# TheClimateCorporation/photon-ml

Measured on AMD Instinct MI355X. Metric: examples/sec/node, logistic L-BFGS 1B×1M-sparse, higher is better.
Workload: dtype bf16; 1 GPU; model=logistic_regression_l2_lbfgs, global_batch=125000000, rows_per_gpu=125000000, features=1000000, nnz_per_row=100, parallelism=dp1, optimizer_state=replicated, layout=tiled

## Files before the change

### photon_ml_amd/ops/csrc/game_kernels.hip

```cpp

#include <hip/hip_runtime.h>
#include <stdint.h>

#include <algorithm>

#ifndef PML_BUILD_ID
#define PML_BUILD_ID "unstamped-build!"
#endif
__attribute__((used)) static const char pml_build_stamp[] = "PML_BUILD_ID=" PML_BUILD_ID;

#define LAUNCH_CHECK()                                         \
  do {                                                         \
    hipError_t e_ = hipGetLastError();                         \
    if (e_ != hipSuccess) return (int)e_;                      \
  } while (0)

#define SCORE_GROUP 16
#define SCORE_THREADS 256
#define SCORE_ROWS_PER_BLOCK (SCORE_THREADS / SCORE_GROUP)

template <bool RE>
__global__ __launch_bounds__(SCORE_THREADS) void score_rows_kernel(
    const long long* __restrict__ indptr, const int* __restrict__ col, const double* __restrict__ val,
    long long n_rows, const double* __restrict__ w, const int* __restrict__ ent,
// ... 90 lines not shown
    for (long long p = lo; p < hi; ++p) {
      const double v = val[p];
      const long long c = col[p];
      if (j < k) acc += v * PT[c * k + j];
    }
    if (j < k) Y[row * k + j] = acc;
  }
}

__device__ __forceinline__ unsigned long long splitmix64(unsigned long long x) {
  x += 0x9E3779B97F4A7C15ull;
  x = (x ^ (x >> 30)) * 0xBF58476D1CE4E5B9ull;
  x = (x ^ (x >> 27)) * 0x94D049BB133111EBull;
  return x ^ (x >> 31);
}

template <typename T>
__global__ __launch_bounds__(256) void downsample_kernel(const T* __restrict__ y, const T* __restrict__ w0,
                                                          const long long* __restrict__ rowid, long long n,
                                                          unsigned long long seed, double rate, int binary,
                                                          T* __restrict__ w) {
  const long long i = (long long)blockIdx.x * 256 + threadIdx.x;
  if (i >= n) return;
  const unsigned long long id = rowid ? (unsigned long long)rowid[i] : (unsigned long long)i;
  const double u = (double)(splitmix64(seed ^ splitmix64(id)) >> 11) * 0x1.0p-53;
  const double wi = (double)w0[i];
  double out;
  if (binary) {
    const bool pos = (double)y[i] >= 0.5;
    out = pos ? wi : (u < rate ? wi / rate : 0.0);
  } else {
    out = u < rate ? wi : 0.0;
  }
  w[i] = (T)out;
}

#define CMP_SEG 8
struct CmpArgs {
  const int* units;
  int col_e, row_col;
  const int* seg;
  int nseg, sbits, key_is_row;
  const uint32_t* pack;
  const void* val;
  const uint16_t* npack;
  const void* nval;
  const int* nbase;
  const unsigned char* keep;
  int* seg_cnt;
  const long long* seg_first;
  const long long* unit_lo;
  uint32_t* opack;
  void* oval;
};

template <typename VT, int PASS>
__global__ __launch_bounds__(256) void tl_compact_kernel(CmpArgs a) {
  const int lane = threadIdx.x & 63;
  const int s = __builtin_amdgcn_readfirstlane(blockIdx.x * 4 + (threadIdx.x >> 6));
  if (s >= a.nseg) return;
  const int* sg = a.seg + 3 * (long long)s;
  const int u = sg[0], r_lo = sg[1], r_hi = sg[2];
  const int* ut = a.units + 6 * (long long)u;
  const long long e_lo = ut[a.col_e];
  const int nw = ut[a.col_e + 1] - ut[a.col_e];
  const int n_lo = ut[4], nn = ut[5] - ut[4];
  const uint32_t row0 = a.row_col >= 0 ? (uint32_t)ut[a.row_col] : 0u;
  const uint32_t smask = (1u << a.sbits) - 1u;
  const VT* val = (const VT*)a.val;
  const VT* nval = (const VT*)a.nval;
  long long ob = PASS ? a.seg_first[s] : 0;
  const long long olo = PASS ? a.unit_lo[u] : 0;
  const unsigned long long below = (1ull << lane) - 1ull;
  int cnt = 0;
  for (int r = r_lo; r < r_hi; ++r) {
    uint32_t p[4];
    VT v[4];
    bool ok[4];
    if (r < nn) {
      const long long q = (long long)n_lo + r;
      const int base = a.nbase[q];
#pragma unroll
      for (int k = 0; k < 4; ++k) {
        const uint32_t p16 = a.npack[q * 256 + 4 * lane + k];
        p[k] = ((uint32_t)(base + (int)(p16 >> a.sbits)) << a.sbits) | (p16 & smask);
        v[k] = nval[q * 256 + 4 * lane + k];
        ok[k] = true;
      }
    } else {
      const int w = r - nn;
#pragma unroll
      for (int k = 0; k < 4; ++k) {
        ok[k] = 256 * w + 64 * k + lane < nw;
        const long long e = e_lo + 256LL * w + 4 * lane + k;
        p[k] = ok[k] ? a.pack[e] : 0u;
        v[k] = ok[k] ? val[e] : (VT)0;
      }
    }
#pragma unroll
    for (int k = 0; k < 4; ++k) {
      const uint32_t row = a.key_is_row ? (p[k] >> a.sbits) : row0 + (p[k] & smask);
      const bool kp = ok[k] && a.keep[row];
      const unsigned long long m = __ballot(kp);
      if (PASS) {
        if (kp) {
          const long long o = ob + __popcll(m & below);
          const long long ph = olo + (o & ~255LL) + ((o & 63) << 2) + ((o & 255) >> 6);
          a.opack[ph] = p[k];
          ((VT*)a.oval)[ph] = v[k];
        }
        ob += __popcll(m);
      } else {
        cnt += __popcll(m);
      }
    }
  }
  if (!PASS && lane == 0) a.seg_cnt[s] = cnt;
}


template <int S, bool STAGE>
__global__ __launch_bounds__(64) void seg_gram_kernel(int B, int n, int dmax, const long long* __restrict__ ents,
                                                      const long long* __restrict__ row_ptr,
                                                      const long long* __restrict__ col_ptr,
                                                      const long long* __restrict__ nip,
                                                      const long long* __restrict__ pos,
                                                      const double* __restrict__ val, double* __restrict__ K) {
  extern __shared__ double img[];
  const int lane = threadIdx.x;
  const long long b = blockIdx.x;
  if (b >= B) return;
  const long long e = ents[b];
  const long long r0 = row_ptr[e];
  const int ne = (int)(row_ptr[e + 1] - r0);
  const long long cb = col_ptr[e];
  const int de = (int)(col_ptr[e + 1] - cb);
  const long long e0 = nip[r0];
  const int enz = (int)(nip[r0 + ne] - e0);
  double* sval = img + (size_t)dmax * S;
  unsigned short* scol = (unsigned short*)(sval + enz);
  int* sptr = (int*)(scol + ((enz + 3) & ~3));
  for (int c = lane; c < de * S; c += 64) img[c] = 0.0;
  if (STAGE) {
    for (int t = lane; t < enz; t += 64) {
      sval[t] = val[e0 + t];
      scol[t] = (unsigned short)(pos[e0 + t] - cb);
    }
    for (int i = lane; i <= ne; i += 64) sptr[i] = (int)(nip[r0 + i] - e0);
  }
  __syncthreads();
  double* Kb = K + b * (long long)n * n;
  for (int i0 = 0; i0 < ne; i0 += S) {
    const int ns = ne - i0 < S ? ne - i0 : S;
    for (int s = 0; s < ns; ++s) {
      if (STAGE) {
        const int ib = sptr[i0 + s], ie = sptr[i0 + s + 1];
        for (int t = ib + lane; t < ie; t += 64) img[(int)scol[t] * S + s] = sval[t];
      } else {
        const long long ib = nip[r0 + i0 + s], ie = nip[r0 + i0 + s + 1];
        for (long long t = ib + lane; t < ie; t += 64) img[(pos[t] - cb) * S + s] = val[t];
      }
    }
    __syncthreads();
    for (int j = lane; j < n; j += 64) {
      double acc[S];
#pragma unroll
      for (int s = 0; s < S; ++s) acc[s] = 0.0;
      if (j < ne) {
        if (STAGE) {
// ... 330 lines not shown
```

### photon_ml_amd/ops/csrc/glm_kernels.hip

```cpp

#include <hip/hip_runtime.h>
#include <stdint.h>
#include <math.h>
#include <algorithm>

#define NB 4096
#define NTHREADS 256
#define VEC 8
#define MAXSEG 1024

#define LAUNCH_CHECK()                                         \
  do {                                                         \
    hipError_t e_ = hipGetLastError();                         \
    if (e_ != hipSuccess) return (int)e_;                      \
  } while (0)

enum LossId { LOSS_LOGISTIC = 0, LOSS_POISSON = 1, LOSS_SQUARED = 2, LOSS_HINGE = 3 };
enum FwdMode { FWD_MARGIN = 0, FWD_VALUE_GRAD = 1, FWD_HV = 2, FWD_DZZ = 3, FWD_LS = 4 };

struct bf16x8 { uint4 u; };

template <typename VT, typename AT> struct Loader;
template <> struct Loader<uint16_t, float> {
  static __device__ __forceinline__ void load8(const uint16_t* __restrict__ p, float* v) {
// ... 746 lines not shown
typedef const __attribute__((address_space(4))) int* const_int_p;

template <typename VT, typename XT, typename AT, bool SQ, int NW, int S, int D>
__device__ __forceinline__ void tl_stream_ring(const uint32_t* __restrict__ pack, const VT* __restrict__ val,
                                               const XT* __restrict__ x, int e_lo, int e_hi, int sbits, AT* acc,
                                               const int* wbase) {
  constexpr int R = S + 1;
  static_assert(D < S && R % (D + 1) == 0, "gathers run ahead of loaded slots; the gather ring divides the slots");
  typedef typename TLValT<VT>::T LT;
  typedef typename TLVals<VT>::Raw Raw;
  const int lane = threadIdx.x & 63;
  const int w = __builtin_amdgcn_readfirstlane(threadIdx.x >> 6);
  const uint32_t smask = (1u << sbits) - 1u;
  const int nr = (e_hi - e_lo + TL_ROUND - 1) / TL_ROUND;
  const int r0 = (nr * w) / NW, r1 = (nr * (w + 1)) / NW;
  if (r0 >= r1) return;
  v4u pk[R];
  Raw vr[R];
  uint32_t bs[R];
  XT xg[D + 1][TL_VEC];
  const int ws = wbase ? 1 : 0;
  const const_int_p wb = (const_int_p)(wbase ? wbase : g_zero_base);
  const int rb0 = e_lo / TL_ROUND;
  auto load_round = [&](int r, v4u& p, Raw& v, uint32_t& b) {
    const int e = e_lo + min(r, r1 - 1) * TL_ROUND + lane * TL_VEC;
    p = ldg_nt((const v4u*)(pack + e));
    v = TLVals<VT>::load(val + e);
    b = (uint32_t)wb[ws * (rb0 + min(r, r1 - 1))];
  };
  const int abl = TL_ABL;
  AT regsum = AT(0);
  auto gather = [&](int r, const v4u& p, uint32_t b, XT* xv) {
    const int e = e_lo + r * TL_ROUND + lane;
#pragma unroll
    for (int k = 0; k < TL_VEC; ++k) {
      const uint32_t key = (e + 64 * k < e_hi) ? b + (p[k] >> sbits) : 0u;
      const bool hot = key < ((uint32_t)abl >> 8) << 10;
      if (abl & 10) xv[k] = XT(1);
      else if ((abl & 32) && hot) xv[k] = XT(1);
      else if ((abl & 64) && __ballot(!hot) == 0ull) xv[k] = XT(1);
      else xv[k] = ldg(x + key);
    }
  };
#pragma unroll
  for (int i = 0; i < S; ++i) {
    load_round(r0 + i, pk[i], vr[i], bs[i]);
    __builtin_amdgcn_sched_barrier(0);
  }
#pragma unroll
  for (int i = 0; i < D; ++i) {
    gather(r0 + i, pk[i], bs[i], xg[i]);
    __builtin_amdgcn_sched_barrier(0);
  }
  for (int r = r0; r < r1; r += R) {
#pragma unroll
    for (int i = 0; i < R; ++i) {
      const int rc = r + i;
      load_round(rc + S, pk[(i + S) % R], vr[(i + S) % R], bs[(i + S) % R]);
      __builtin_amdgcn_sched_barrier(0);
      gather(rc + D, pk[(i + D) % R], bs[(i + D) % R], xg[(i + D) % (D + 1)]);
      __builtin_amdgcn_sched_barrier(0);
      LT v[TL_VEC];
      TLVals<VT>::get(vr[i], v);
      const int e = e_lo + rc * TL_ROUND + lane;
#pragma unroll
      for (int k = 0; k < TL_VEC; ++k) {
        const bool in = (e + 64 * k < e_hi) && (rc < r1);
        const AT vv = SQ ? static_cast<AT>(v[k]) * static_cast<AT>(v[k]) : static_cast<AT>(v[k]);
        AT add;
        if (abl & 4) add = in ? static_cast<AT>(static_cast<float>(v[k]) * static_cast<float>(xg[i % (D + 1)][k]))
                              : AT(0);
        else add = in ? vv * static_cast<AT>(xg[i % (D + 1)][k]) : AT(0);
        if (abl & 1) regsum += add;
        else atomicAdd(&acc[in ? (pk[i][k] & smask) : 0u], add);
      }
      __builtin_amdgcn_sched_barrier(0);
    }
  }
  if (abl & 1) atomicAdd(&acc[lane], regsum);
}

template <typename T> __device__ __forceinline__ T lane_bcast(T v, int src) { return __shfl(v, src, 64); }

template <typename VT, typename XT, typename AT, bool SQ, int NW, int S = 2>
__device__ __forceinline__ void tl_stream_narrow(const uint16_t* __restrict__ npk, const VT* __restrict__ nvl,
                                                 const int* __restrict__ nbs, int n_lo, int n_hi, int sbits,
                                                 const XT* __restrict__ x, AT* acc) {
  constexpr int R = S + 1;
  typedef typename TLValT<VT>::T LT;
  typedef typename TLVals<VT>::Raw Raw;
  const int lane = threadIdx.x & 63;
  const int w = __builtin_amdgcn_readfirstlane(threadIdx.x >> 6);
  const int nr = n_hi - n_lo;
  const int r0 = n_lo + (nr * w) / NW, r1 = n_lo + (nr * (w + 1)) / NW;
  if (r0 >= r1) return;
  const uint32_t smask = (1u << sbits) - 1u;
  const const_int_p bp = (const_int_p)nbs;
  v2u pks[R];
  Raw vs[R];
  XT xs[R];
  const int abl = TL_ABL;
  AT regsum = AT(0);
  auto issue = [&](int r, int base, v2u& pk, Raw& v, XT& xw) {
    const size_t e = (size_t)min(r, r1 - 1) * TL_ROUND + lane * TL_VEC;
    pk = ldg_nt((const v2u*)(npk + e));
    v = TLVals<VT>::load(nvl + e);
    xw = (abl & 18) ? XT(1) : ldg(x + base + lane);
  };
#pragma unroll
  for (int i = 0; i < S; ++i) {
    issue(r0 + i, bp[min(r0 + i, r1 - 1)], pks[i], vs[i], xs[i]);
    __builtin_amdgcn_sched_barrier(0);
  }
  int nb = bp[min(r0 + S, r1 - 1)];
  for (int r = r0; r < r1; r += R) {
#pragma unroll
    for (int i = 0; i < R; ++i) {
      const int rc = r + i;
      issue(rc + S, nb, pks[(i + S) % R], vs[(i + S) % R], xs[(i + S) % R]);
      nb = bp[min(rc + S + 1, r1 - 1)];
      __builtin_amdgcn_sched_barrier(0);
      const bool live = rc < r1;
      LT v[TL_VEC];
      TLVals<VT>::get(vs[i], v);
      const v2u pk = pks[i];
      const uint32_t p[TL_VEC] = {pk.x & 0xffffu, pk.x >> 16, pk.y & 0xffffu, pk.y >> 16};
#pragma unroll
      for (int k = 0; k < TL_VEC; ++k) {
        const XT xv = (abl & 16) ? xs[i] : lane_bcast(xs[i], (int)(p[k] >> sbits));
        const AT vv = SQ ? static_cast<AT>(v[k]) * static_cast<AT>(v[k]) : static_cast<AT>(v[k]);
        AT add;
        if (abl & 4) add = live ? static_cast<AT>(static_cast<float>(v[k]) * static_cast<float>(xv)) : AT(0);
        else add = live ? vv * static_cast<AT>(xv) : AT(0);
        if (abl & 1) regsum += add + AT(p[k] & smask);
        else atomicAdd(&acc[live ? (p[k] & smask) : 0u], add);
      }
      __builtin_amdgcn_sched_barrier(0);
    }
  }
  if (abl & 1) atomicAdd(&acc[lane], regsum);
}

template <typename VT, typename XT, typename AT, bool SQ, int U, int NW, int P>
__device__ __forceinline__ void tl_stream(const uint32_t* __restrict__ pack, const VT* __restrict__ val,
                                          const XT* __restrict__ x, int e_lo, int e_hi, int sbits, AT* acc,
                                          const int* wbase = nullptr) {
  if (P == 1) tl_stream_p1<VT, XT, AT, SQ, U, NW>(pack, val, x, e_lo, e_hi, sbits, acc);
  else if (P == 2) tl_stream_wide<VT, XT, AT, SQ, NW, 2>(pack, val, x, e_lo, e_hi, sbits, acc);
  else if (P == 3) tl_stream_ring<VT, XT, AT, SQ, NW, 2, 0>(pack, val, x, e_lo, e_hi, sbits, acc, wbase);
  else if (P == 5) tl_stream_ring<VT, XT, AT, SQ, NW, 3, 1>(pack, val, x, e_lo, e_hi, sbits, acc, wbase);
  else if (P == 6) tl_stream_ring<VT, XT, AT, SQ, NW, 5, 2>(pack, val, x, e_lo, e_hi, sbits, acc, wbase);
  else tl_stream_p0<VT, XT, AT, SQ, U, NW>(pack, val, x, e_lo, e_hi, sbits, acc);
}

struct TLNarrow { const uint16_t* pack; const void* val; const int* base; const int* wbase; };

template <typename VT, typename XT, typename RT, typename AT, int MAXR, int U, int NW, int P>
__device__ __forceinline__ void tl_fwd_block(int b, int row_lo, int nrows, int e_lo, int e_hi, int n_lo, int n_hi,
                                             int rbits, const uint32_t* __restrict__ pack,
                                             const VT* __restrict__ val, const TLNarrow& nar,
                                             const XT* __restrict__ x, const FwdArgs<XT, RT>& a,
                                             double* __restrict__ stats, AT (*acc)[MAXR], double* red) {
  const int R = 1 << rbits;
  for (int i = threadIdx.x; i < R; i += NW * 64)
#pragma unroll
    for (int w = 0; w < NW; ++w) acc[w][i] = AT(0);
  __syncthreads();
  if (n_hi > n_lo)
    tl_stream_narrow<VT, XT, AT, false, NW, (P >= 5 ? 4 : 2)>(nar.pack, (const VT*)nar.val, nar.base, n_lo, n_hi,
                                                              rbits, x,
                                            acc[threadIdx.x >> 6]);
  tl_stream<VT, XT, AT, false, U, NW, P>(pack, val, x, e_lo, e_hi, rbits, acc[threadIdx.x >> 6], nar.wbase);
  __syncthreads();
  double F = 0.0, S = 0.0;
  for (int r = threadIdx.x; r < nrows; r += NW * 64) {
    double z = static_cast<double>(acc[0][r]);
#pragma unroll
    for (int w = 1; w < NW; ++w) z += static_cast<double>(acc[w][r]);
    const int s = row_lo + r;
    fwd_finish(a, s, z, fwd_prefetch(a, s), F, S);
  }
  if (stats) {
    block_sum2_nw<NW>(F, S, red);
    if (threadIdx.x == 0) { stats[2 * b] = F; stats[2 * b + 1] = S; }
  }
}

template <typename VT, typename XT, typename RT, typename AT, int MAXR, int U, int NW, int P>
__global__ __launch_bounds__(NW * 64) void tl_fwd_kernel(const int* __restrict__ blk, int rbits,
                                                          const uint32_t* __restrict__ pack,
                                                          const VT* __restrict__ val, TLNarrow nar,
                                                          const XT* __restrict__ x, FwdArgs<XT, RT> a,
                                                          double* __restrict__ stats,
                                                          const unsigned char* __restrict__ live) {
  __shared__ AT acc[NW][MAXR];
  __shared__ double red[2 * NW];
  const int b = blockIdx.x;
  if (live && !live[b]) return;
  const int* q = blk + 6 * b;
  tl_fwd_block<VT, XT, RT, AT, MAXR, U, NW, P>(b, q[0], q[1], q[2], q[3], q[4], q[5], rbits, pack, val, nar, x, a,
                                              stats, acc, red);
}

template <typename VT, typename XT, typename RT, typename AT, int MAXR, int U, int NW, int P>
__global__ __launch_bounds__(NW * 64) void tl_fwd_multi_kernel(const int* __restrict__ blk, int rbits,
                                                                const unsigned long long* __restrict__ ptrs,
                                                                const XT* __restrict__ x, FwdArgs<XT, RT> a,
                                                                double* __restrict__ stats,
                                                                const unsigned char* __restrict__ live) {
  __shared__ AT acc[NW][MAXR];
  __shared__ double red[2 * NW];
  const int b = blockIdx.x;
  if (live && !live[b]) return;
  const int* q = blk + 8 * b;
  const unsigned long long* pc = ptrs + 6 * q[0];
  const TLNarrow nar = {(const uint16_t*)pc[2], (const void*)pc[3], (const int*)pc[4], (const int*)pc[5]};
  tl_fwd_block<VT, XT, RT, AT, MAXR, U, NW, P>(b, q[1], q[2], q[3], q[4], q[6], q[7], rbits, (const uint32_t*)pc[0],
                                              (const VT*)pc[1], nar, x + q[5], a, stats, acc, red);
}

template <typename VT, typename XT, typename AT, bool SQ, int MAXR, int U, int NW, int P>
__device__ __forceinline__ void tl_t_item(int tile, int e_lo, int e_hi, int part, int n_lo, int n_hi, int cbits,
                                          const uint32_t* __restrict__ pack, const VT* __restrict__ val,
                                          const TLNarrow& nar, const XT* __restrict__ x, double* __restrict__ G,
                                          int dim, double* __restrict__ parts, AT (*acc)[MAXR]) {
  const int C = 1 << cbits;
  for (int i = threadIdx.x; i < C; i += NW * 64)
#pragma unroll
    for (int w = 0; w < NW; ++w) acc[w][i] = AT(0);
  __syncthreads();
  if (n_hi > n_lo)
    tl_stream_narrow<VT, XT, AT, SQ, NW, (P >= 5 ? 4 : 2)>(nar.pack, (const VT*)nar.val, nar.base, n_lo, n_hi,
                                                           cbits, x,
                                         acc[threadIdx.x >> 6]);
  tl_stream<VT, XT, AT, SQ, U, NW, P>(pack, val, x, e_lo, e_hi, cbits, acc[threadIdx.x >> 6], nar.wbase);
  __syncthreads();
  const int c0 = tile << cbits;
  for (int c = threadIdx.x; c < C; c += NW * 64) {
    double s = static_cast<double>(acc[0][c]);
#pragma unroll
    for (int w = 1; w < NW; ++w) s += static_cast<double>(acc[w][c]);
    if (part < 0) {
      if (c0 + c < dim) G[c0 + c] += s;
    } else {
      parts[(size_t)part * C + c] = s;
    }
  }
}

template <typename VT, typename XT, typename AT, bool SQ, int MAXR, int U, int NW, int P>
__global__ __launch_bounds__(NW * 64) void tl_t_kernel(const int* __restrict__ items, int cbits,
                                                        const uint32_t* __restrict__ pack,
                                                        const VT* __restrict__ val, TLNarrow nar,
                                                        const XT* __restrict__ x, double* __restrict__ G, int dim,
                                                        double* __restrict__ parts,
                                                        const unsigned char* __restrict__ live) {
  __shared__ AT acc[NW][MAXR];
  if (live && !live[blockIdx.x]) return;
  const int* q = items + 6 * blockIdx.x;
  tl_t_item<VT, XT, AT, SQ, MAXR, U, NW, P>(q[0], q[1], q[2], q[3], q[4], q[5], cbits, pack, val, nar, x, G, dim,
                                            parts, acc);
}

template <typename VT, typename XT, typename AT, bool SQ, int MAXR, int U, int NW, int P>
__global__ __launch_bounds__(NW * 64) void tl_t_multi_kernel(const int* __restrict__ items, int cbits,
                                                              const unsigned long long* __restrict__ ptrs,
                                                              const XT* __restrict__ x, double* __restrict__ G,
                                                              int dim, double* __restrict__ parts,
                                                              const unsigned char* __restrict__ live,
                                                              const int* __restrict__ gate) {
  __shared__ AT acc[NW][MAXR];
  if (gate && *gate == 0) return;
  if (live && !live[blockIdx.x]) return;
  const int* q = items + 8 * blockIdx.x;
  const unsigned long long* pc = ptrs + 6 * q[0];
  const TLNarrow nar = {(const uint16_t*)pc[2], (const void*)pc[3], (const int*)pc[4], (const int*)pc[5]};
  tl_t_item<VT, XT, AT, SQ, MAXR, U, NW, P>(q[1], q[2], q[3], q[4], q[6], q[7], cbits, (const uint32_t*)pc[0],
                                            (const VT*)pc[1], nar, x + q[5], G, dim, parts, acc);
}

__device__ __forceinline__ double rows_sum64(const double* __restrict__ src, int C, int r0, int r1, int c,
                                             double* sh) {
  const int w = threadIdx.x >> 6, lane = threadIdx.x & 63;
  const int n = r1 - r0;
  const int q0 = r0 + (n * w) / 4, q1 = r0 + (n * (w + 1)) / 4;
  double s0 = 0.0, s1 = 0.0, s2 = 0.0, s3 = 0.0;
  if (c < C) {
    int r = q0;
    for (; r + 3 < q1; r += 4) {
      s0 += src[(size_t)r * C + c];
      s1 += src[(size_t)(r + 1) * C + c];
      s2 += src[(size_t)(r + 2) * C + c];
      s3 += src[(size_t)(r + 3) * C + c];
    }
    for (; r < q1; ++r) s0 += src[(size_t)r * C + c];
  }
  sh[w * 64 + lane] = (s0 + s1) + (s2 + s3);
  __syncthreads();
  return (sh[lane] + sh[64 + lane]) + (sh[128 + lane] + sh[192 + lane]);
}

__global__ __launch_bounds__(NTHREADS) void tl_t_combine1_kernel(const int* __restrict__ cu, int cbits,
                                                                 const double* __restrict__ parts,
                                                                 double* __restrict__ l1,
                                                                 const unsigned char* __restrict__ live_mt) {
  __shared__ double sh[NTHREADS];
  const int u = blockIdx.x;
  if (live_mt && !live_mt[cu[3 * u]]) return;
  const int C = 1 << cbits;
  const int c = blockIdx.y * 64 + (threadIdx.x & 63);
  const double s = rows_sum64(parts, C, cu[3 * u + 1], cu[3 * u + 2], c, sh);
  if (threadIdx.x < 64 && c < C) l1[(size_t)u * C + c] = s;
}

__global__ __launch_bounds__(NTHREADS) void tl_t_combine2_kernel(const int* __restrict__ mt_tiles,
                                                                 const int* __restrict__ mt_ptr, int cbits,
                                                                 const double* __restrict__ l1,
// ... 2454 lines not shown
```

### photon_ml_amd/ops/device.py

```python
from __future__ import annotations

import ctypes
import os
import threading
from dataclasses import dataclass
from typing import List, Optional, Sequence

import numpy as np
import scipy.sparse as sp
import torch

from ..data.matrix import LabeledData
from .native import SegChunkDesc, check, require_glm_lib, stream_handle
from .reference import GLMComputable
from .tiled import DEFAULT_ITEM_ENTRIES, TLFwdChunk, TLTChunk, tl_supported
from ..utils.timing import phase, trace_range

H2D_GATE = threading.Event()

LAYOUTS = ("auto", "tiled", "segmented")


def resolve_layout(layout: str, dim: int, chunk_rows: int) -> str:
    import os
# ... 150 lines not shown
        if os.environ.get("PML_CHECK_KERNEL_INPUTS", "0") == "1":
            self.validate()

    def validate(self):
        from .tiled import il_phys
        for c, (f, t) in enumerate(zip(self.csr, self.csc)):
            if f.kind != "tl":
                continue
            m = self.row_starts[c + 1] - self.row_starts[c]
            b = f.blk.cpu().to(torch.int64)
            if f.nblk and (int(b[:, 0].min()) < 0 or int((b[:, 0] + b[:, 1]).max()) > m
                           or int(b[:, 1].max()) > (1 << f.rbits)):
                raise ValueError(f"chunk {c}: forward block rows out of range")
            q = 256 if f.il else 4
            end = b[:, 2] + (b[:, 3] - b[:, 2] + q - 1) // q * q if f.il else (b[:, 3] + 3) // 4 * 4
            if f.nblk and (int(b[:, 2].min()) < 0 or int(end.max()) > f.pack.numel()):
                raise ValueError(f"chunk {c}: forward block window outside the stream")
            if f.il and f.nblk and bool((b[:, 2] % 256 != 0).any()):
                raise ValueError(f"chunk {c}: interleaved forward windows not round-aligned")
            ncols = int(self.dim) - self.col_lo[c]
            self._validate_narrow(c, f, b, ncols, "forward")
            pk, _ = f.logical()
            p = pk.cpu().to(torch.int64)
            wb = getattr(f, "wbase", None)
            if wb is not None and wb.numel() and int(wb.min()) < 0:
                raise ValueError(f"chunk {c}: negative wide-round base")
            if p.numel() and int((p >> f.rbits).max()) >= ncols:
                raise ValueError(f"chunk {c}: forward gather index >= column window")
            counts = f.unit_counts().cpu()
            blk_rows = torch.repeat_interleave(b[:, 1], counts)
            if p.numel() and bool(((p & ((1 << f.rbits) - 1)) >= blk_rows).any()):
                raise ValueError(f"chunk {c}: forward LDS slot >= block rows")
            it = t.items.cpu().to(torch.int64)
            if t.nitems:
                if int(it[:, 1].min()) < 0 or int(it[:, 2].max()) > t.pack.numel():
                    raise ValueError(f"chunk {c}: transpose item window outside the stream")
                if int(it[:, 3].max()) >= max(t.nparts, 1) and t.nparts:
                    raise ValueError(f"chunk {c}: transpose partial-row slot out of range")
                self._validate_narrow(c, t, it, m, "transpose")
                tp, _ = t.logical()
                q = tp.cpu().to(torch.int64) & 0xFFFFFFFF
                if q.numel() and int((q >> t.cbits).max()) >= m:
                    raise ValueError(f"chunk {c}: transpose gather row >= chunk rows")
                cols = (torch.repeat_interleave(it[:, 0], t.unit_counts().cpu()) << t.cbits) + (q & ((1 << t.cbits) - 1))
                if q.numel() and int(cols.max()) >= t.dim:
                    raise ValueError(f"chunk {c}: transpose column >= dim")
        if self.parts.numel() < max([c.parts_needed for c in self.csr + self.csc] + [1]):
            raise ValueError("partial-row scratch too small")
        self._validate_multi()
        return True

    def _validate_multi(self):
        mb = getattr(self, "_multi", None)
        if mb is not None and not isinstance(mb, str):
            t = self._multi_blk.cpu().to(torch.int64)
            for c, ch in enumerate(self.csr):
                r = t[t[:, 0] == c]
                if ch.il and r.shape[0] and (int(r[:, 3].min()) < 0 or int((r[:, 3] + (r[:, 4] - r[:, 3] + 255) // 256 * 256).max())
                                   > ch.pack.numel() or int(r[:, 7].max()) > ch.nbase.numel() * (ch.n_narrow_rounds > 0)):
                    raise ValueError(f"chunk {c}: shard-wide forward table outside the chunk's streams")
        mt = getattr(self, "_multi_t", None)
        if mt is not None and not isinstance(mt, str):
            if self.parts.numel() < mt.parts_needed:
                raise ValueError("partial-row scratch too small for the shard-wide transpose")
            t = mt.items.cpu().to(torch.int64)
            for c, ch in enumerate(self.csc):
                r = t[t[:, 0] == c]
                if ch.il and r.shape[0] and (int(r[:, 2].min()) < 0 or int((r[:, 2] + (r[:, 3] - r[:, 2] + 255) // 256 * 256).max())
                                   > ch.pack.numel() or int(r[:, 7].max()) > ch.nbase.numel() * (ch.n_narrow_rounds > 0)):
                    raise ValueError(f"chunk {c}: shard-wide transpose table outside the chunk's streams")

    @staticmethod
    def _validate_narrow(c: int, ch, table: torch.Tensor, xlen: int, what: str):
        if table.shape[0] == 0:
            return
        n_lo, n_hi = table[:, 4], table[:, 5]
        nrounds = ch.nbase.numel() if ch.n_narrow_rounds else 0
        if bool((n_hi < n_lo).any()) or int(n_hi.max()) > nrounds or bool((n_lo[1:] != n_hi[:-1]).any()):
            raise ValueError(f"chunk {c}: {what} narrow round ranges inconsistent")
        if nrounds:
            base = ch.nbase.cpu().to(torch.int64)
            if ch.npack.numel() < 256 * nrounds or ch.nval.numel() < 256 * nrounds:
                raise ValueError(f"chunk {c}: {what} narrow stream shorter than its rounds")
            if int(base.min()) < 0 or int(base.max()) + 64 > xlen:
                raise ValueError(f"chunk {c}: {what} narrow key window outside the gathered vector")

    @staticmethod
    def from_labeled(data: LabeledData, device="cuda", precision: str = "f64", chunk_rows: int = 1 << 20,
                     relabel: bool = True, layout: str = "auto", item_entries: Optional[int] = None,
                     col_windows: bool = False):
        if col_windows:
            relabel = False
        prec = PRECISIONS[precision]
        vdt = VAL_DTYPE[prec]
        dev = torch.device(device)
        x = data.x.tocsr()
        n, d = x.shape
        if dev.type == "cuda" and n and resolve_layout(layout, d, chunk_rows) == "tiled":
            return DeviceGLMData._from_labeled_device(x, data, dev, precision, chunk_rows, relabel, item_entries,
                                                      col_windows)
        if hasattr(x, "to_scipy"):
            x = x.to_scipy()
        old_of_new = None
        from ..parallel.dist import is_dist
        shared = relabel and is_dist() and not col_windows
        if shared or (relabel and x.nnz > 0):
            counts = np.bincount(x.indices, minlength=d).astype(np.int64)
            if shared:
                import torch.distributed as tdist
                from ..parallel.sharding import comm_device
                ct = torch.from_numpy(counts).to(comm_device())
                tdist.all_reduce(ct)
                counts = ct.cpu().numpy()
            old_of_new_np = np.argsort(-counts, kind="stable")
            new_of_old_np = np.empty(d, dtype=np.int64)
            new_of_old_np[old_of_new_np] = np.arange(d)
            x = sp.csr_matrix((x.data, new_of_old_np[x.indices], x.indptr), shape=x.shape)
            old_of_new = torch.from_numpy(old_of_new_np)
        starts = list(range(0, n, chunk_rows)) + [n]
        if n == 0:
            starts = [0, 0]
        csr, csc = [], []
        col_lo = []
        wins = []
        align = _window_align(chunk_rows, precision)
        for a, b in zip(starts[:-1], starts[1:]):
            xc = x[a:b]
            if col_windows and xc.nnz:
                lo, hi = int(xc.indices.min()), int(xc.indices.max()) + 1
                lo -= lo % align
            else:
                lo, hi = 0, d
            wins.append((lo, hi))
        dmax = max([hi - lo for lo, hi in wins] + [1])
        layout = resolve_layout(layout, dmax, chunk_rows)
        cbits = None
        if layout == "tiled" and not col_windows and item_entries is None:
            from .tiled import shard_t_config
            cbits, item_entries = shard_t_config(int(x.nnz), n, d, chunk_rows)
        for (a, b), (lo, hi) in zip(zip(starts[:-1], starts[1:]), wins):
            xc = x[a:b]
            col_lo.append(lo)
            if lo != 0 or hi != d:
                xc = sp.csr_matrix((xc.data, xc.indices - lo, xc.indptr), shape=(b - a, hi - lo))
            dc = hi - lo
            if layout == "tiled":
                rp = torch.from_numpy((xc.indptr - xc.indptr[0]).astype(np.int64)).to(dev)
                col = torch.from_numpy(xc.indices.astype(np.int64)).to(dev)
                val = torch.from_numpy(xc.data.astype(np.float64)).to(dev).to(vdt)
                csr.append(TLFwdChunk(rp, col, val, dc))
                csc.append(TLTChunk(rp, col, val, dc, chunk_rows, cbits=cbits, item_entries=item_entries))
                continue
            sp_ = (xc.indptr - xc.indptr[0]).astype(np.int32)
            csr.append(SegChunk(sp_, torch.from_numpy(xc.indices.astype(np.int32)),
                                torch.from_numpy(xc.data.astype(np.float64)).to(vdt), dev, forward=True))
            xt = xc.tocsc()
            xt.sort_indices()
            xc = xc.copy()
            csc.append(SegChunk(xt.indptr.astype(np.int32), torch.from_numpy(xt.indices.astype(np.int32)),
                                torch.from_numpy(xt.data.astype(np.float64)).to(vdt), dev))
        out = DeviceGLMData(csr, csc, starts, torch.from_numpy(data.y), torch.from_numpy(data.offsets),
                            torch.from_numpy(data.weights), d, precision, dev, old_of_new)
        out.col_lo = col_lo
        return out

    @staticmethod
# ... 886 lines not shown
```

### photon_ml_amd/ops/tiled.py

```python
from __future__ import annotations

import ctypes
import math
import os
from typing import Optional, Sequence, Tuple

import numpy as np
import torch

from .native import TLFwdDesc, TLTDesc

TL_MAXBITS = 12
TL_MAXBITS_F64 = 11
TL_MINBITS = 5
DEFAULT_RBITS = int(os.environ.get("PML_TL_RBITS", 10))
DEFAULT_CBITS = int(os.environ.get("PML_TL_CBITS", 10))
DEFAULT_ITEM_ENTRIES = 1 << 18
_PAD = 8
COMBINE_SEG = 16


XCD_GROUPS = int(os.environ.get("PML_TL_XCD", "0"))


def xcd_order(chunk_of_item: np.ndarray, groups: int) -> np.ndarray:
    stream = np.asarray(chunk_of_item) % groups
    lists = [np.flatnonzero(stream == k) for k in range(groups)]
    longest = max(len(l) for l in lists)
    grid = np.full((longest, groups), -1, dtype=np.int64)
    for k, l in enumerate(lists):
        grid[: len(l), k] = l
    order = grid.reshape(-1)
    return order[order >= 0]


def combine_seg(k: int) -> int:
    return max(COMBINE_SEG, int(math.ceil(math.sqrt(k))))
IL_ROUND = 256
TL_VEC = 4
INTERLEAVE = int(os.environ.get("PML_TL_IL", "1"))
NARROW = int(os.environ.get("PML_TL_NARROW", "1"))
NARROW_W = 64
WIDE_BASE = int(os.environ.get("PML_TL_WIDE_BASE", "1"))


def narrow_width(sbits: int) -> int:
    return min(NARROW_W, 1 << max(16 - sbits, 0))


def _bits(n: int) -> int:
    return max(1, int(n - 1).bit_length())


def _cap(want: int, f64: bool) -> int:
    return min(want, TL_MAXBITS_F64 if f64 else TL_MAXBITS)


F64_WIDE_RBITS = 11


def default_rbits(dim: int, f64: bool) -> int:
    if f64 and dim >= (1 << 16) and "PML_TL_RBITS" not in os.environ:
        return F64_WIDE_RBITS
    return DEFAULT_RBITS


def fwd_bits(dim: int, f64: bool = False, want: Optional[int] = None) -> Optional[int]:
    r = min(_cap(default_rbits(dim, f64) if want is None else want, f64), 32 - _bits(dim))
    return r if r >= TL_MINBITS else None


def t_bits(chunk_rows: int, f64: bool = False, want: Optional[int] = None) -> Optional[int]:
    c = min(_cap(DEFAULT_CBITS if want is None else want, f64), 32 - _bits(chunk_rows))
    return c if c >= TL_MINBITS else None


SPARSE_TILE_ENTRIES = 1 << 16


def shard_t_config(nnz: int, n_rows: int, dim: int, chunk_rows: int):
    if "PML_TL_CBITS" in os.environ or "PML_TL_ITEM_ENTRIES" in os.environ or n_rows <= 0 or dim < (1 << 16):
        return None, None
    per_tile = (nnz / n_rows) * min(chunk_rows, n_rows) / math.ceil(dim / 1024)
    if per_tile < SPARSE_TILE_ENTRIES:
        return 11, 1 << 17
    return None, None


def tl_supported(dim: int, chunk_rows: int) -> bool:
    return fwd_bits(dim) is not None and t_bits(chunk_rows) is not None


def _to_u32_bits(x64: torch.Tensor) -> torch.Tensor:
    return torch.where(x64 >= (1 << 31), x64 - (1 << 32), x64).to(torch.int32)


def _pad(t: torch.Tensor) -> torch.Tensor:
    return torch.cat([t, torch.zeros(_PAD, dtype=t.dtype, device=t.device)]).contiguous()


def il_phys(e_lo: torch.Tensor, n: torch.Tensor) -> torch.Tensor:
    e_lo = e_lo.to(torch.int64)
    n = n.to(torch.int64)
    tot = int(n.sum())
    unit = torch.repeat_interleave(torch.arange(n.numel(), device=n.device), n)
    j = torch.arange(tot, device=n.device) - (torch.cumsum(n, 0) - n)[unit]
    t = j & (IL_ROUND - 1)
    return e_lo[unit] + (j - t) + ((t & 63) << 2) + (t >> 6)


def _interleave(pack: torch.Tensor, val: torch.Tensor, n: torch.Tensor):
    n = n.to(torch.int64)
    padded = (n + IL_ROUND - 1) // IL_ROUND * IL_ROUND
    new_lo = torch.cumsum(padded, 0) - padded
    total = int(padded.sum()) + _PAD
    phys = il_phys(new_lo, n)
    p = torch.zeros(total, dtype=pack.dtype, device=pack.device)
    v = torch.zeros(total, dtype=val.dtype, device=val.device)
    p[phys] = pack
    v[phys] = val
    return p, v, new_lo


def _empty_narrow(val: torch.Tensor):
    dev = val.device
    return (torch.zeros(IL_ROUND, dtype=torch.int16, device=dev), torch.zeros(IL_ROUND, dtype=val.dtype, device=dev),
            torch.zeros(1, dtype=torch.int32, device=dev))


def split_narrow(pack: torch.Tensor, val: torch.Tensor, n: torch.Tensor, sbits: int, xlen: int, enable: bool = True):
    dev = pack.device
    n = n.to(torch.int64)
    U = n.numel()
    gcount = n // IL_ROUND
    W = narrow_width(sbits)
    ok = enable and NARROW and W >= 16 and xlen >= NARROW_W and int(gcount.sum()) > 0
    if not ok:
        z = torch.zeros(U, dtype=torch.int64, device=dev)
        return (pack, val, n, *_empty_narrow(val), z)
    starts = torch.cumsum(n, 0) - n
    gu = torch.repeat_interleave(torch.arange(U, device=dev), gcount)
    gi = torch.arange(gu.numel(), device=dev) - (torch.cumsum(gcount, 0) - gcount)[gu]
    gs = starts[gu] + IL_ROUND * gi
    key = pack >> sbits
    first, last = key[gs], key[gs + IL_ROUND - 1]
    base = torch.clamp(first, max=xlen - NARROW_W)
    nar = (last - base) < W
    gs_n, base = gs[nar], base[nar]
    idx = gs_n[:, None] + torch.arange(IL_ROUND, device=dev)[None, :]
    p16 = ((key[idx] - base[:, None]) << sbits) | (pack[idx] & ((1 << sbits) - 1))
    il = lambda t: t.reshape(-1, TL_VEC, 64).transpose(1, 2).reshape(-1)
    npack = il(torch.where(p16 >= 32768, p16 - 65536, p16).to(torch.int16)).contiguous()
    nval = il(val[idx]).contiguous()
    nbase = base.to(torch.int32).contiguous()
    cs = torch.zeros(nar.numel() + 1, dtype=torch.int64, device=dev)
    torch.cumsum(nar.to(torch.int64), 0, out=cs[1:])
    ge = torch.cumsum(gcount, 0)
    nrounds = cs[ge] - cs[ge - gcount]
    keep = torch.ones(pack.numel(), dtype=torch.bool, device=dev)
    keep[idx.reshape(-1)] = False
    del idx, p16
    return pack[keep], val[keep], n - IL_ROUND * nrounds, npack, nval, nbase, nrounds



def narrow_logical(npack: torch.Tensor, nval: torch.Tensor, nbase: torch.Tensor, r_lo, r_hi, sbits: int):
    r = torch.arange(int(r_lo), int(r_hi), device=npack.device)
    if not r.numel():
        return torch.zeros(0, dtype=torch.int64, device=npack.device), nval[:0]
    ph = (r[:, None] * IL_ROUND + torch.arange(IL_ROUND, device=npack.device)[None, :]).reshape(-1, 64, TL_VEC)
    ph = ph.transpose(1, 2).reshape(-1)
    p16 = npack[ph].to(torch.int64) & 0xFFFF
    base = nbase[r].to(torch.int64).repeat_interleave(IL_ROUND)
    return (((p16 >> sbits) + base) << sbits) | (p16 & ((1 << sbits) - 1)), nval[ph]


class _NarrowMixin:

    wbase = None

    def _set_narrow(self, npack, nval, nbase):
        from .native import TLNarrow
        self.npack, self.nval, self.nbase = npack, nval, nbase
        self.nar = TLNarrow(npack.data_ptr(), nval.data_ptr(), nbase.data_ptr(),
                            None if self.wbase is None else self.wbase.data_ptr())

    @property
    def n_narrow_rounds(self) -> int:
        t = self._table()
        return int((t[:, 5] - t[:, 4]).sum()) if t.shape[0] else 0

    def unit_counts(self) -> torch.Tensor:
        t = self._table().to(torch.int64)
        lo, hi = self._ew
        return (t[:, hi] - t[:, lo]) + IL_ROUND * (t[:, 5] - t[:, 4])

    def narrow_window(self, r_lo: int, r_hi: int):
        return narrow_logical(self.npack, self.nval, self.nbase, r_lo, r_hi, self._sbits)

    def _logical_all(self, wide_pack, wide_val):
        t = self._table().to(torch.int64)
        dev = wide_pack.device
        lo, hi = self._ew
        nn = IL_ROUND * (t[:, 5] - t[:, 4])
        nw = t[:, hi] - t[:, lo]
        if int(nn.sum()) == 0:
            return wide_pack, wide_val
        npk, nvl = narrow_logical(self.npack, self.nval, self.nbase, 0, int(t[:, 5].max()), self._sbits)
        U = t.shape[0]
        nu = torch.repeat_interleave(torch.arange(U, device=dev), nn.to(dev))
        nj = torch.arange(int(nn.sum()), device=dev) - (torch.cumsum(nn, 0) - nn).to(dev)[nu]
        npos = t[:, 4].to(dev)[nu] * IL_ROUND + nj
        wu = torch.repeat_interleave(torch.arange(U, device=dev), nw.to(dev))
        unit = torch.cat([nu, wu])
        order = torch.sort(unit, stable=True).indices
        wp = wide_pack.to(torch.int64) & 0xFFFFFFFF if wide_pack.dtype == torch.int32 else wide_pack.to(torch.int64)
        pk = torch.cat([npk[npos], wp])[order]
        vl = torch.cat([nvl[npos], wide_val])[order]
        return pk, vl


class TLFwdChunk(_NarrowMixin):

    kind = "tl"

    def __init__(self, rowptr: torch.Tensor, col: torch.Tensor, val: torch.Tensor, dim: int,
                 rbits: Optional[int] = None, il: Optional[int] = None):
        dev = val.device
        self.il = INTERLEAVE if il is None else int(il)
        rowptr = rowptr.to(dev, torch.int64)
        col = col.to(dev, torch.int64)
        m = rowptr.numel() - 1
        f64 = val.dtype == torch.float64
        self.rbits = fwd_bits(dim, f64, rbits)
        if self.rbits is None:
            raise ValueError(f"tiled forward layout cannot pack dim={dim}")
        want = _cap(default_rbits(dim, f64) if rbits is None else rbits, f64)
        use_base = bool(self.il) and WIDE_BASE and want > self.rbits
        if use_base:
            self.rbits = want
        R = 1 << self.rbits
        kbits = _bits(dim) + self.rbits
        nnz = col.numel()
        rows = torch.repeat_interleave(torch.arange(m, device=dev), rowptr[1:] - rowptr[:-1]) if nnz else \
            torch.zeros(0, dtype=torch.int64, device=dev)
        pack = (col << self.rbits) | (rows & (R - 1))
        key = ((rows >> self.rbits) << kbits) | pack
        key, perm = torch.sort(key, stable=True)
        nblk = (m + R - 1) // R
        b = torch.arange(nblk, device=dev)
        lo = b * R
        hi = torch.clamp(lo + R, max=m)
        e_lo, e_hi = rowptr[lo], rowptr[hi]
        self._sbits, self._ew = self.rbits, (2, 3)
        n_lo = n_hi = torch.zeros(nblk, dtype=torch.int64, device=dev)
        if self.il:
            wp, wv, wn, npk, nvl, nbs, nr = split_narrow(key & ((1 << kbits) - 1), val[perm], e_hi - e_lo,
                                                         self.rbits, dim)
            del key, perm
            if use_base:
                wp = self._rebase(wp, wn)
                if wp is None:
                    del wv, npk, nvl, nbs
                    self.__init__(rowptr, col, val, dim, fwd_bits(dim, f64, rbits), il)
                    return
            self.pack, self.val, e_lo = _interleave(_to_u32_bits(wp), wv, wn)
            e_hi = e_lo + wn
            n_hi = torch.cumsum(nr, 0)
# ... 217 lines not shown
        part[order[multi_tile]] = np.arange(int(multi_tile.sum()))
        km = k[k > 1]
        plo = np.cumsum(km) - km
        sg = np.maximum(COMBINE_SEG, np.ceil(np.sqrt(km)).astype(np.int64)) if len(km) else km
        nu = -(-km // sg)
        u_tile = np.repeat(np.arange(len(km)), nu)
        u_first = np.repeat(plo, nu) + np.repeat(sg, nu) * (np.arange(int(nu.sum())) - np.repeat(np.cumsum(nu) - nu, nu))
        u_last = np.minimum(u_first + np.repeat(sg, nu), np.repeat(plo + km, nu))
        self.nitems, self.nparts, self.ncu, self.nmt = n, int(km.sum()), int(nu.sum()), len(km)
        rows = np.column_stack([it[:, 0], it[:, 1], it[:, 2], it[:, 3], part, it[:, 4], it[:, 5],
                                it[:, 6]]).astype(np.int32)
        src = src_all if tile_range is None else src_all[in_range]
        if XCD_GROUPS > 1 and n > XCD_GROUPS:
            xo = xcd_order(it[:, 0], XCD_GROUPS)
            rows, src = rows[xo], src[xo]
        self._src = torch.from_numpy(src.astype(np.int64)).to(dev)
        self.items = torch.tensor(rows.reshape(-1, 8), device=dev)
        self.mt_tiles = torch.tensor(np.r_[ts[starts][k > 1], 0].astype(np.int32)[: max(self.nmt, 1)], device=dev)
        self.mt_ptr = torch.tensor(np.r_[0, np.cumsum(nu)].astype(np.int32), device=dev)
        self.cu = torch.tensor(np.column_stack([u_tile, u_first, u_last]).astype(np.int32).reshape(-1, 3)
                               if self.ncu else np.zeros((1, 3), np.int32), device=dev)
        self.ptrs = stream_ptr_table(chunks, dev)
        self._chunks = list(chunks)
        self.desc = TLTMultiDesc(self.items.data_ptr(), n, self.cbits, self.ptrs.data_ptr(),
                                 self.mt_tiles.data_ptr(), self.mt_ptr.data_ptr(), self.nmt, dim,
                                 self.cu.data_ptr(), self.ncu, self.nparts, self.il)

    @property
    def parts_needed(self) -> int:
        return (self.nparts + self.ncu) << self.cbits

    def restreamed(self, chunks: Sequence["TLTChunk"]) -> "TLTMulti":
        import copy
        from .native import TLTMultiDesc
        dev = self.items.device
        cat = torch.cat([ch.items[: ch.nitems].to(torch.int64) for ch in chunks]) if chunks else None
        rows = self.items.to(torch.int64).clone()
        if self.nitems:
            sel = cat[self._src]
            rows[:, 2:4] = sel[:, 1:3]
            rows[:, 6:8] = sel[:, 4:6]
        new = copy.copy(self)
        new.items = rows.to(torch.int32).contiguous()
        new.ptrs = stream_ptr_table(chunks, dev)
        new._chunks = list(chunks)
        d = self.desc
        new.desc = TLTMultiDesc(new.items.data_ptr(), d.nitems, d.cbits, new.ptrs.data_ptr(), d.mt_tiles, d.mt_ptr,
                                d.nmt, d.dim, d.cu, d.ncu, d.nparts_total, d.il)
        return new

    def emulate_rmatvec(self, r: torch.Tensor, square: bool = False) -> torch.Tensor:
        C = 1 << self.cbits
        dim = self.desc.dim
        ntiles = (dim + C - 1) // C
        G = torch.zeros(ntiles * C, dtype=torch.float64)
        parts = torch.zeros((max(self.nparts, 1), C), dtype=torch.float64)
        r = r.to(torch.float64).cpu()
        for c, tile, e_lo, e_hi, part, rb, n_lo, n_hi in self.items.cpu().tolist():
            ch = self._chunks[c]
            pk, vl = ch.window(e_lo, e_hi)
            npk, nvl = ch.narrow_window(n_lo, n_hi)
            p = torch.cat([npk.cpu(), pk.to(torch.int64).cpu() & 0xFFFFFFFF])
            v = torch.cat([nvl.cpu(), vl.cpu()]).to(torch.float64)
            if square:
                v = v * v
            acc = torch.zeros(C, dtype=torch.float64).index_add_(0, p & (C - 1), v * r[rb + (p >> self.cbits)])
            if part < 0:
                G[tile * C:(tile + 1) * C] += acc
            else:
                parts[part] = acc
        cu = self.cu.cpu().tolist()
        l1 = [parts[a:b].sum(0) for _, a, b in cu[: self.ncu]]
        mp = self.mt_ptr.cpu().tolist()
        for t, tile in enumerate(self.mt_tiles.cpu().tolist()[: self.nmt]):
            s = torch.zeros(C, dtype=torch.float64)
            for u in range(mp[t], mp[t + 1]):
                s += l1[u]
            G[tile * C:(tile + 1) * C] += s
        return G[:dim]


def stream_ptr_table(chunks, device) -> torch.Tensor:
    wb = lambda ch: 0 if getattr(ch, "wbase", None) is None else ch.wbase.data_ptr()
    return torch.tensor([[ch.pack.data_ptr(), ch.val.data_ptr(), ch.npack.data_ptr(), ch.nval.data_ptr(),
                          ch.nbase.data_ptr(), wb(ch)] for ch in chunks], dtype=torch.int64,
                        device=device).reshape(-1)


CMP_SEG = 8


def _cmp_segments(ch, narrow: bool):
    cache = ch.__dict__.setdefault("_cmp_seg", {})
    if cache.get(narrow) is not None:
        return cache[narrow]
    t = ch._table().to(torch.int64)
    dev = t.device
    lo, hi = ch._ew
    nn = t[:, 5] - t[:, 4]
    R = (t[:, hi] - t[:, lo] + IL_ROUND - 1) // IL_ROUND + (nn if narrow else 0)
    ns = (R + CMP_SEG - 1) // CMP_SEG
    S = int(ns.sum())
    su = torch.repeat_interleave(torch.arange(t.shape[0], device=dev), ns, output_size=S)
    first = (torch.cumsum(ns, 0) - ns)[su]
    r_lo = (torch.arange(S, device=dev) - first) * CMP_SEG
    r_hi = torch.minimum(r_lo + CMP_SEG, R[su])
    if not narrow:
        r_lo, r_hi = r_lo + nn[su], r_hi + nn[su]
    seg = torch.stack([su, r_lo, r_hi], 1).to(torch.int32).contiguous()
    cache[narrow] = (seg, su, first, S, IL_ROUND * int(nn.sum()))
    return cache[narrow]


class RowCompaction:

    def __init__(self, ch, keep: torch.Tensor, forward: bool, filter_narrow: bool = False):
        from .native import CmpArgs, check, require_game_lib, stream_handle
        if not ch.il:
            raise ValueError("row-sampled copies need the interleaved layout")
        self.ch, self.keep, self.forward = ch, keep, forward
        dev = ch.pack.device
        self.filter_narrow = bool(filter_narrow)
        seg, su, first, S, self.n_narrow = _cmp_segments(ch, self.filter_narrow)
        table = ch._table()
        lo, hi = ch._ew
        self.seg_cnt = torch.zeros(max(S, 1), dtype=torch.int32, device=dev)
        self._keep_alive = (seg, table, keep)
        self.args = CmpArgs(table.data_ptr(), lo, 0 if forward else -1, seg.data_ptr(), S, ch._sbits,
                            0 if forward else 1, ch.pack.data_ptr(), ch.val.data_ptr(), ch.npack.data_ptr(),
                            ch.nval.data_ptr(), ch.nbase.data_ptr(), keep.data_ptr(), self.seg_cnt.data_ptr(),
                            None, None, None, None)
        self.lib, self.stream = require_game_lib(), stream_handle(dev)
        self.vbytes = ch.val.element_size()
        if S:
            check(self.lib.pml_tl_compact(0, self.vbytes, ctypes.byref(self.args), self.stream), "tl_compact count")
        cnt = self.seg_cnt[:S].to(torch.int64)
        U = table.shape[0]
        self.unit_cnt = torch.zeros(U, dtype=torch.int64, device=dev).index_add_(0, su, cnt)
        padded = (self.unit_cnt + IL_ROUND - 1) // IL_ROUND * IL_ROUND
        self.unit_lo = (torch.cumsum(padded, 0) - padded).contiguous()
        excl = torch.cumsum(cnt, 0) - cnt
        self.seg_first = (excl - excl[first]).contiguous() if S else excl
        self.total, self.kept = padded.sum(), self.unit_cnt.sum()

    def finish(self, total: int, kept: int):
        import copy
        from .native import TLFwdDesc, TLTDesc, check
        ch = self.ch
        dev = ch.pack.device
        opack = torch.zeros(total + _PAD, dtype=torch.int32, device=dev)
        oval = torch.zeros(total + _PAD, dtype=ch.val.dtype, device=dev)
        a = self.args
        a.seg_first, a.unit_lo = self.seg_first.data_ptr(), self.unit_lo.data_ptr()
        a.opack, a.oval = opack.data_ptr(), oval.data_ptr()
        if a.nseg:
            check(self.lib.pml_tl_compact(1, self.vbytes, ctypes.byref(a), self.stream), "tl_compact write")
        lo, hi = ch._ew
        table = ch._table().to(torch.int64).clone()
        table[:, lo] = self.unit_lo
        table[:, hi] = self.unit_lo + self.unit_cnt
        if self.filter_narrow:
            table[:, 4:6] = 0
        table = table.to(torch.int32).contiguous()
        nc = copy.copy(ch)
        nc._cmp_seg = {}
        nc.pack, nc.val = opack, oval
        if self.filter_narrow:
            nc._set_narrow(*_empty_narrow(oval))
            nc.nnz = kept
        else:
            nc.nnz = kept + self.n_narrow
        if self.forward:
            nc.blk = table
            nc.desc = TLFwdDesc(table.data_ptr(), nc.nblk, nc.rbits, opack.data_ptr(), oval.data_ptr(), 1, nc.nar)
        else:
            nc.items = table
            nc.desc = TLTDesc(table.data_ptr(), nc.nitems, nc.cbits, opack.data_ptr(), oval.data_ptr(),
                              nc.mt_tiles.data_ptr(), nc.mt_ptr.data_ptr(), nc.nmt, nc.dim, nc.cu.data_ptr(), nc.ncu,
                              nc.nparts, 1, nc.nar)
        return nc
```

Measured before the change: 3.266 billion examples/sec.

## Interleave narrow-stream keys and bf16 values into fused 16-byte per-lane records

For bf16 data, the narrow stream's 16-bit packed keys and bf16 values are concatenated into one record per lane, four keys followed by four values. The narrow streaming kernel then loads both with a single 16-byte non-temporal load instead of two separate 8-byte loads from different arrays. The compaction kernel and the host-side logical decoding are updated to read the fused layout. The aim is fewer memory transactions and better access locality, at the cost of extra layout paths and stricter validation.

```diff
diff --git a/photon_ml_amd/ops/csrc/game_kernels.hip b/photon_ml_amd/ops/csrc/game_kernels.hip
--- a/photon_ml_amd/ops/csrc/game_kernels.hip
+++ b/photon_ml_amd/ops/csrc/game_kernels.hip
@@ -196,9 +196,10 @@
       const int base = a.nbase[q];
 #pragma unroll
       for (int k = 0; k < 4; ++k) {
-        const uint32_t p16 = a.npack[q * 256 + 4 * lane + k];
+        const long long pe = nval ? q * 256 + 4 * lane + k : q * 512 + 8 * lane + k;
+        const uint32_t p16 = a.npack[pe];
         p[k] = ((uint32_t)(base + (int)(p16 >> a.sbits)) << a.sbits) | (p16 & smask);
-        v[k] = nval[q * 256 + 4 * lane + k];
+        v[k] = nval ? nval[pe] : ((const VT*)a.npack)[pe + 4];
         ok[k] = true;
       }
     } else {
diff --git a/photon_ml_amd/ops/csrc/glm_kernels.hip b/photon_ml_amd/ops/csrc/glm_kernels.hip
--- a/photon_ml_amd/ops/csrc/glm_kernels.hip
+++ b/photon_ml_amd/ops/csrc/glm_kernels.hip
@@ -852,7 +852,28 @@
 
 template <typename T> __device__ __forceinline__ T lane_bcast(T v, int src) { return __shfl(v, src, 64); }
 
-template <typename VT, typename XT, typename AT, bool SQ, int NW, int S = 2>
+template <typename VT, bool FUSED> struct TLNarrowSlot {
+  typedef typename TLVals<VT>::Raw Raw;
+  v2u pk;
+  Raw v;
+  __device__ __forceinline__ void load(const uint16_t* npk, const VT* nvl, size_t e) {
+    pk = ldg_nt((const v2u*)(npk + e));
+    v = TLVals<VT>::load(nvl + e);
+  }
+  __device__ __forceinline__ v2u packs() const { return pk; }
+  __device__ __forceinline__ Raw vals() const { return v; }
+};
+template <> struct TLNarrowSlot<uint16_t, true> {
+  typedef v2u Raw;
+  v4u rec;
+  __device__ __forceinline__ void load(const uint16_t* npk, const uint16_t*, size_t e) {
+    rec = ldg_nt((const v4u*)(npk + 2 * e));
+  }
+  __device__ __forceinline__ v2u packs() const { v2u p; p.x = rec.x; p.y = rec.y; return p; }
+  __device__ __forceinline__ Raw vals() const { v2u u; u.x = rec.z; u.y = rec.w; return u; }
+};
+
+template <typename VT, typename XT, typename AT, bool SQ, int NW, int S = 2, bool FUSED = false>
 __device__ __forceinline__ void tl_stream_narrow(const uint16_t* __restrict__ npk, const VT* __restrict__ nvl,
                                                  const int* __restrict__ nbs, int n_lo, int n_hi, int sbits,
                                                  const XT* __restrict__ x, AT* acc) {
@@ -866,20 +887,19 @@
   if (r0 >= r1) return;
   const uint32_t smask = (1u << sbits) - 1u;
   const const_int_p bp = (const_int_p)nbs;
-  v2u pks[R];
-  Raw vs[R];
+  typedef TLNarrowSlot<VT, FUSED> Slot;
+  Slot sl[R];
   XT xs[R];
   const int abl = TL_ABL;
   AT regsum = AT(0);
-  auto issue = [&](int r, int base, v2u& pk, Raw& v, XT& xw) {
+  auto issue = [&](int r, int base, Slot& s, XT& xw) {
     const size_t e = (size_t)min(r, r1 - 1) * TL_ROUND + lane * TL_VEC;
-    pk = ldg_nt((const v2u*)(npk + e));
-    v = TLVals<VT>::load(nvl + e);
+    s.load(npk, nvl, e);
     xw = (abl & 18) ? XT(1) : ldg(x + base + lane);
   };
 #pragma unroll
   for (int i = 0; i < S; ++i) {
-    issue(r0 + i, bp[min(r0 + i, r1 - 1)], pks[i], vs[i], xs[i]);
+    issue(r0 + i, bp[min(r0 + i, r1 - 1)], sl[i], xs[i]);
     __builtin_amdgcn_sched_barrier(0);
   }
   int nb = bp[min(r0 + S, r1 - 1)];
@@ -887,13 +907,13 @@
 #pragma unroll
     for (int i = 0; i < R; ++i) {
       const int rc = r + i;
-      issue(rc + S, nb, pks[(i + S) % R], vs[(i + S) % R], xs[(i + S) % R]);
+      issue(rc + S, nb, sl[(i + S) % R], xs[(i + S) % R]);
       nb = bp[min(rc + S + 1, r1 - 1)];
       __builtin_amdgcn_sched_barrier(0);
       const bool live = rc < r1;
       LT v[TL_VEC];
-      TLVals<VT>::get(vs[i], v);
-      const v2u pk = pks[i];
+      TLVals<VT>::get(sl[i].vals(), v);
+      const v2u pk = sl[i].packs();
       const uint32_t p[TL_VEC] = {pk.x & 0xffffu, pk.x >> 16, pk.y & 0xffffu, pk.y >> 16};
 #pragma unroll
       for (int k = 0; k < TL_VEC; ++k) {
@@ -925,6 +945,18 @@
 
 struct TLNarrow { const uint16_t* pack; const void* val; const int* base; const int* wbase; };
 
+template <typename VT, typename XT, typename AT, bool SQ, int NW, int S>
+__device__ __forceinline__ void tl_narrow(const TLNarrow& nar, int n_lo, int n_hi, int sbits,
+                                          const XT* __restrict__ x, AT* acc) {
+  if constexpr (sizeof(VT) == 2) {
+    if (nar.val == nullptr) {
+      tl_stream_narrow<VT, XT, AT, SQ, NW, S, true>(nar.pack, nullptr, nar.base, n_lo, n_hi, sbits, x, acc);
+      return;
+    }
+  }
+  tl_stream_narrow<VT, XT, AT, SQ, NW, S, false>(nar.pack, (const VT*)nar.val, nar.base, n_lo, n_hi, sbits, x, acc);
+}
+
 template <typename VT, typename XT, typename RT, typename AT, int MAXR, int U, int NW, int P>
 __device__ __forceinline__ void tl_fwd_block(int b, int row_lo, int nrows, int e_lo, int e_hi, int n_lo, int n_hi,
                                              int rbits, const uint32_t* __restrict__ pack,
@@ -937,9 +969,7 @@
     for (int w = 0; w < NW; ++w) acc[w][i] = AT(0);
   __syncthreads();
   if (n_hi > n_lo)
-    tl_stream_narrow<VT, XT, AT, false, NW, (P >= 5 ? 4 : 2)>(nar.pack, (const VT*)nar.val, nar.base, n_lo, n_hi,
-                                                              rbits, x,
-                                            acc[threadIdx.x >> 6]);
+    tl_narrow<VT, XT, AT, false, NW, (P >= 5 ? 4 : 2)>(nar, n_lo, n_hi, rbits, x, acc[threadIdx.x >> 6]);
   tl_stream<VT, XT, AT, false, U, NW, P>(pack, val, x, e_lo, e_hi, rbits, acc[threadIdx.x >> 6], nar.wbase);
   __syncthreads();
   double F = 0.0, S = 0.0;
@@ -1000,9 +1030,7 @@
     for (int w = 0; w < NW; ++w) acc[w][i] = AT(0);
   __syncthreads();
   if (n_hi > n_lo)
-    tl_stream_narrow<VT, XT, AT, SQ, NW, (P >= 5 ? 4 : 2)>(nar.pack, (const VT*)nar.val, nar.base, n_lo, n_hi,
-                                                           cbits, x,
-                                         acc[threadIdx.x >> 6]);
+    tl_narrow<VT, XT, AT, SQ, NW, (P >= 5 ? 4 : 2)>(nar, n_lo, n_hi, cbits, x, acc[threadIdx.x >> 6]);
   tl_stream<VT, XT, AT, SQ, U, NW, P>(pack, val, x, e_lo, e_hi, cbits, acc[threadIdx.x >> 6], nar.wbase);
   __syncthreads();
   const int c0 = tile << cbits;
diff --git a/photon_ml_amd/ops/device.py b/photon_ml_amd/ops/device.py
--- a/photon_ml_amd/ops/device.py
+++ b/photon_ml_amd/ops/device.py
@@ -256,6 +256,9 @@
             base = ch.nbase.cpu().to(torch.int64)
             if ch.npack.numel() < 256 * nrounds or ch.nval.numel() < 256 * nrounds:
                 raise ValueError(f"chunk {c}: {what} narrow stream shorter than its rounds")
+            if ch.fused and (ch.nrec.numel() < 512 * nrounds or ch.val.element_size() != 2
+                             or not ch.nrec.is_contiguous()):
+                raise ValueError(f"chunk {c}: {what} fused narrow records need 2-byte values, 16 B per lane and round")
             if int(base.min()) < 0 or int(base.max()) + 64 > xlen:
                 raise ValueError(f"chunk {c}: {what} narrow key window outside the gathered vector")
 
diff --git a/photon_ml_amd/ops/tiled.py b/photon_ml_amd/ops/tiled.py
--- a/photon_ml_amd/ops/tiled.py
+++ b/photon_ml_amd/ops/tiled.py
@@ -41,6 +41,7 @@
 INTERLEAVE = int(os.environ.get("PML_TL_IL", "1"))
 NARROW = int(os.environ.get("PML_TL_NARROW", "1"))
 NARROW_W = 64
+FUSE = int(os.environ.get("PML_TL_FUSE", "1"))
 WIDE_BASE = int(os.environ.get("PML_TL_WIDE_BASE", "1"))
 
 
@@ -152,6 +153,9 @@
     il = lambda t: t.reshape(-1, TL_VEC, 64).transpose(1, 2).reshape(-1)
     npack = il(torch.where(p16 >= 32768, p16 - 65536, p16).to(torch.int16)).contiguous()
     nval = il(val[idx]).contiguous()
+    if FUSE and val.dtype == torch.bfloat16:
+        npack = torch.cat([npack.view(-1, TL_VEC), nval.view(torch.int16).view(-1, TL_VEC)], 1).reshape(-1)
+        nval = None
     nbase = base.to(torch.int32).contiguous()
     cs = torch.zeros(nar.numel() + 1, dtype=torch.int64, device=dev)
     torch.cumsum(nar.to(torch.int64), 0, out=cs[1:])
@@ -167,23 +171,36 @@
 def narrow_logical(npack: torch.Tensor, nval: torch.Tensor, nbase: torch.Tensor, r_lo, r_hi, sbits: int):
     r = torch.arange(int(r_lo), int(r_hi), device=npack.device)
     if not r.numel():
-        return torch.zeros(0, dtype=torch.int64, device=npack.device), nval[:0]
+        return torch.zeros(0, dtype=torch.int64, device=npack.device), nval[:0].reshape(-1)
     ph = (r[:, None] * IL_ROUND + torch.arange(IL_ROUND, device=npack.device)[None, :]).reshape(-1, 64, TL_VEC)
     ph = ph.transpose(1, 2).reshape(-1)
-    p16 = npack[ph].to(torch.int64) & 0xFFFF
+    rl, rh = int(r_lo) * IL_ROUND, int(r_hi) * IL_ROUND
+    ph = ph - rl
+    p16 = npack.reshape(-1, TL_VEC)[rl // TL_VEC:rh // TL_VEC].reshape(-1)[ph].to(torch.int64) & 0xFFFF
     base = nbase[r].to(torch.int64).repeat_interleave(IL_ROUND)
-    return (((p16 >> sbits) + base) << sbits) | (p16 & ((1 << sbits) - 1)), nval[ph]
+    return ((((p16 >> sbits) + base) << sbits) | (p16 & ((1 << sbits) - 1)),
+            nval.reshape(-1, TL_VEC)[rl // TL_VEC:rh // TL_VEC].reshape(-1)[ph])
 
 
 class _NarrowMixin:
 
     wbase = None
+
+    nrec = None
 
     def _set_narrow(self, npack, nval, nbase):
         from .native import TLNarrow
+        self.nrec = npack if nval is None else None
+        if nval is None:
+            rec = npack.view(-1, 2 * TL_VEC)
+            npack, nval = rec[:, :TL_VEC], rec[:, TL_VEC:].view(torch.bfloat16)
         self.npack, self.nval, self.nbase = npack, nval, nbase
-        self.nar = TLNarrow(npack.data_ptr(), nval.data_ptr(), nbase.data_ptr(),
+        self.nar = TLNarrow(npack.data_ptr(), None if self.fused else nval.data_ptr(), nbase.data_ptr(),
                             None if self.wbase is None else self.wbase.data_ptr())
+
+    @property
+    def fused(self) -> bool:
+        return self.nrec is not None
 
     @property
     def n_narrow_rounds(self) -> int:
@@ -567,9 +584,9 @@
 
 def stream_ptr_table(chunks, device) -> torch.Tensor:
     wb = lambda ch: 0 if getattr(ch, "wbase", None) is None else ch.wbase.data_ptr()
-    return torch.tensor([[ch.pack.data_ptr(), ch.val.data_ptr(), ch.npack.data_ptr(), ch.nval.data_ptr(),
-                          ch.nbase.data_ptr(), wb(ch)] for ch in chunks], dtype=torch.int64,
-                        device=device).reshape(-1)
+    return torch.tensor([[ch.pack.data_ptr(), ch.val.data_ptr(), ch.npack.data_ptr(),
+                          0 if ch.fused else ch.nval.data_ptr(), ch.nbase.data_ptr(), wb(ch)] for ch in chunks],
+                        dtype=torch.int64, device=device).reshape(-1)
 
 
 CMP_SEG = 8
@@ -613,7 +630,8 @@
         self._keep_alive = (seg, table, keep)
         self.args = CmpArgs(table.data_ptr(), lo, 0 if forward else -1, seg.data_ptr(), S, ch._sbits,
                             0 if forward else 1, ch.pack.data_ptr(), ch.val.data_ptr(), ch.npack.data_ptr(),
-                            ch.nval.data_ptr(), ch.nbase.data_ptr(), keep.data_ptr(), self.seg_cnt.data_ptr(),
+                            None if ch.fused else ch.nval.data_ptr(), ch.nbase.data_ptr(), keep.data_ptr(),
+                            self.seg_cnt.data_ptr(),
                             None, None, None, None)
         self.lib, self.stream = require_game_lib(), stream_handle(dev)
         self.vbytes = ch.val.element_size()
```

After: 3.319 billion examples/sec, median of 6. 1.02x the previous value.
